# arhix52/Strelka

Hardware: AMD Instinct MI355X
Metric: Mray/s (higher is better)
Workload: dtype f32; 1 GPU; kitchen stand-in (SURVEY 8d C3): 1724134 unique triangles, 2022 instances of 153 meshes, 4 rect + 1 distant light, 60/25/10/5 % diffuse/glossy/metal/glass; resolution=1920x1080, bounces=4, spp=64, tile=32, world_size=1, parallelism=single GPU, rays_per_frame=839862650

## Files before the change

### strelka_amd/csrc/skh_device.h

```cpp
#pragma once
#include <hip/hip_runtime.h>
#include <stdint.h>
#include "skh_libm.h"
#include "skh_lshape.h"

namespace skh
{

struct v3
{
    float x, y, z;
};
struct v4
{
    float x, y, z, w;
};

#define SKH_DI static __device__ __forceinline__

SKH_DI v3 mk3(float x, float y, float z)
{
    v3 r;
    r.x = x;
    r.y = y;
// ... 331 lines not shown
    return norm;
}
SKH_DI void fill_light_data(const Light& l, const v3& hitPoint, LightSample& d)
{
    d.area = calc_light_area(l);
    d.normal = calc_light_normal(l, hitPoint);
    const v3 toLight = d.pointOnLight - hitPoint;
    const float lenToLight = length(toLight);
    d.L = toLight / lenToLight;
    d.distToLight = lenToLight;
}
struct SphQuad
{
    v3 o, x, y, z;
    float z0, z0sq, x0, y0, y0sq, x1, y1, y1sq, b0, b1, b0sq, k, S;
};
SKH_DI SphQuad sph_quad_init(const Light& l, const v3& o)
{
    SphQuad q;
    const v3 ex = mk3(l.points[1]) - mk3(l.points[0]);
    const v3 ey = mk3(l.points[3]) - mk3(l.points[0]);
    const v3 s = mk3(l.points[0]);
    const float exl = length(ex);
    const float eyl = length(ey);
    q.o = o;
    q.x = ex / exl;
    q.y = ey / eyl;
    q.z = cross(q.x, q.y);
    const v3 d = s - o;
    q.z0 = dot(d, q.z);
    if (q.z0 > 0)
    {
        q.z = q.z * -1.0f;
        q.z0 *= -1.0f;
    }
    q.z0sq = q.z0 * q.z0;
    q.x0 = dot(d, q.x);
    q.y0 = dot(d, q.y);
    q.x1 = q.x0 + exl;
    q.y1 = q.y0 + eyl;
    q.y0sq = q.y0 * q.y0;
    q.y1sq = q.y1 * q.y1;
    const v3 v00 = mk3(q.x0, q.y0, q.z0), v01 = mk3(q.x0, q.y1, q.z0), v10 = mk3(q.x1, q.y0, q.z0),
             v11 = mk3(q.x1, q.y1, q.z0);
    const v3 n0 = normalize(cross(v00, v10));
    const v3 n1 = normalize(cross(v10, v11));
    const v3 n2 = normalize(cross(v11, v01));
    const v3 n3 = normalize(cross(v01, v00));
    const float g0 = skm::acosf_(-dot(n0, n1));
    const float g1 = skm::acosf_(-dot(n1, n2));
    const float g2 = skm::acosf_(-dot(n2, n3));
    const float g3 = skm::acosf_(-dot(n3, n0));
    q.b0 = n0.z;
    q.b1 = n2.z;
    q.b0sq = q.b0 * q.b0;
    q.k = 2.0f * SKH_PI - g2 - g3;
    q.S = g0 + g1 - q.k;
    return q;
}
SKH_DI v3 sph_quad_sample(const SphQuad& q, float u, float v)
{
    const float au = u * q.S + q.k;
    const float fu = (skm::cosf_(au) * q.b0 - q.b1) / skm::sinf_(au);
    float cu = 1.0f / sqrtf(fu * fu + q.b0sq) * (fu > 0.0f ? 1.0f : -1.0f);
    cu = clampf(cu, -1.0f, 1.0f);
    float xu = -(cu * q.z0) / sqrtf(1.0f - cu * cu);
    xu = clampf(xu, q.x0, q.x1);
    const float d = sqrtf(xu * xu + q.z0sq);
    const float h0 = q.y0 / sqrtf(d * d + q.y0sq);
    const float h1 = q.y1 / sqrtf(d * d + q.y1sq);
    const float hv = h0 + v * (h1 - h0);
    const float hv2 = hv * hv;
    const float eps = 1e-5f;
    const float yv = (hv < 1.0f - eps) ? (hv * d) / sqrtf(1 - hv2) : q.y1;
    return (q.o + xu * q.x + yv * q.y + q.z0 * q.z);
}
SKH_DI float get_light_pdf(const Light& l, const v3& lightHitPoint, const v3& surfaceHitPoint)
{
    switch (l.type)
    {
    case 0: {
        LightSample d;
        d.pointOnLight = lightHitPoint;
        fill_light_data(l, surfaceHitPoint, d);
        return d.distToLight * d.distToLight / (dot(-d.L, d.normal) * d.area);
    }
    case 2:
        return 1.0f / (4.0f * SKH_PI);
    case 3:
        return 1.0f / (2.0f * SKH_PI * (1.0f - skm::cosf_(l.halfAngle)));
    default:
        break;
    }
    return 0.0f;
}
SKH_DI LightSample sample_rect_light_uniform(const Light& l, float ux, float uy, const v3& hitPoint)
{
    LightSample d;
    const v3 e1 = mk3(l.points[1]) - mk3(l.points[0]);
    const v3 e2 = mk3(l.points[3]) - mk3(l.points[0]);
    d.pointOnLight = mk3(l.points[0]) + e1 * ux + e2 * uy;
    fill_light_data(l, hitPoint, d);
    d.pdf = d.distToLight * d.distToLight / (-dot(d.L, d.normal) * d.area);
    return d;
}
SKH_DI LightSample sample_rect_light(const Light& l, float ux, float uy, const v3& hitPoint)
{
    LightSample d;
    const v3 e1 = mk3(l.points[1]) - mk3(l.points[0]);
    const v3 e2 = mk3(l.points[3]) - mk3(l.points[0]);
    const SphQuad quad = sph_quad_init(l, hitPoint);
    if (quad.S <= 0.0f)
    {
        d.pdf = 0.0f;
        d.pointOnLight = mk3(l.points[0]) + e1 * ux + e2 * uy;
        fill_light_data(l, hitPoint, d);
        return d;
    }
    if (quad.S < 1e-3f)
    {
        d.pointOnLight = mk3(l.points[0]) + e1 * ux + e2 * uy;
        fill_light_data(l, hitPoint, d);
        d.pdf = d.distToLight * d.distToLight / (-dot(d.L, d.normal) * d.area);
        return d;
    }
    d.pointOnLight = sph_quad_sample(quad, ux, uy);
    fill_light_data(l, hitPoint, d);
    d.pdf = 1.0f / quad.S;
    return d;
}
SKH_DI void create_coordinate_system(const v3& N, v3& Nt, v3& Nb)
{
    if (fabsf(N.x) > fabsf(N.y))
    {
        const float invLen = 1.0f / sqrtf(N.x * N.x + N.z * N.z);
        Nt = mk3(-N.z * invLen, 0.0f, N.x * invLen);
    }
    else
    {
        const float invLen = 1.0f / sqrtf(N.y * N.y + N.z * N.z);
        Nt = mk3(0.0f, N.z * invLen, -N.y * invLen);
// ... 543 lines not shown
    EV_ABSORB = 0,
    EV_DIFFUSE = 1,
    EV_GLOSSY = 2,
    EV_SPECULAR = 4,
    EV_REFLECTION = 8,
    EV_TRANSMISSION = 16
};
struct Material
{
    uint32_t type;
    float base_color[3];
    float roughness, metallic, specular, ior;
    uint32_t base_color_texture, normal_texture;
    float reserved[6];
};
struct BsdfSample
{
    v3 k2, bsdf_over_pdf;
    float pdf;
    int event_type;
};
struct BsdfEval
{
    v3 bsdf_diffuse, bsdf_glossy;
    float pdf;
};
SKH_DI v3 cosine_hemisphere(float u1, float u2, float& cosTheta)
{
    const float r = sqrtf(u1);
    const float phi = 2.0f * SKH_PI * u2;
// ... 27 lines not shown
    const v3 T2 = cross(Vh, T1);
    const float r = sqrtf(u1);
    const float phi = 2.0f * SKH_PI * u2;
    const float t1 = r * skm::cosf_(phi);
    float t2 = r * skm::sinf_(phi);
    const float s = 0.5f * (1.0f + Vh.z);
    t2 = (1.0f - s) * sqrtf(fmaxf(0.0f, 1.0f - t1 * t1)) + s * t2;
    const v3 Nh = t1 * T1 + t2 * T2 + sqrtf(fmaxf(0.0f, 1.0f - t1 * t1 - t2 * t2)) * Vh;
    return normalize(mk3(alpha * Nh.x, alpha * Nh.y, fmaxf(0.0f, Nh.z)));
}
struct PbrTerms
{
    v3 diffuse_albedo, f0;
    float alpha, p_spec;
};
SKH_DI PbrTerms pbr_terms(const Material& m)
{
    PbrTerms t;
    const v3 base = mk3(m.base_color[0], m.base_color[1], m.base_color[2]);
    const float metallic = clampf(m.metallic, 0.0f, 1.0f);
    t.diffuse_albedo = base * (1.0f - metallic);
    const float d = 0.08f * m.specular;
    t.f0 = mk3(d) + (base - mk3(d)) * metallic;
    const float r = fmaxf(m.roughness, 0.05f);
    t.alpha = r * r;
    t.p_spec = 0.5f + 0.5f * metallic;
    return t;
}
SKH_DI void pbr_eval_local(const PbrTerms& t, const v3& wo, const v3& wi, v3& fd, v3& fs, float& pdf)
{
    fd = mk3(0.0f);
    fs = mk3(0.0f);
    pdf = 0.0f;
    if (wo.z <= 0.0f || wi.z <= 0.0f)
        return;
    const v3 h = normalize(wo + wi);
    const float oh = fmaxf(dot(wo, h), 0.0f);
    const v3 F = schlick3(t.f0, oh);
    const float D = ggx_D(t.alpha, h.z);
// ... 356 lines not shown
SKH_DI bool hair_frame(const v3& normal, const v3& tangent_u, v3& X, v3& Y, v3& Z)
{
    const float tl = dot(tangent_u, tangent_u);
    if (!(tl > 0.0f))
        return false;
    X = tangent_u * (1.0f / sqrtf(tl));
    const v3 z = normal - X * dot(normal, X);
    const float zl = dot(z, z);
    if (!(zl > 1e-12f))
        return false;
    Z = z * (1.0f / sqrtf(zl));
    Y = cross(Z, X);
    return true;
}

template <bool HAIR>
SKH_DI void bsdf_sample(const Material& m, const v3& stN, const v3& stNg, const v3& stT, const v3& k1, float xi0, float xi1, float xi2,
                        float xi3, bool inside, BsdfSample& out, const HairConst* hc = nullptr )
{
    v3 N = stN, Ng = stNg;
    if (dot(Ng, k1) < 0.0f)
    {
        N = -N;
        Ng = -Ng;
    }
    v3 b1, b2;
    onb_from_z(N, b1, b2);
    const v3 wo = mk3(dot(k1, b1), dot(k1, b2), dot(k1, N));
    out.k2 = mk3(0.0f);
    out.bsdf_over_pdf = mk3(0.0f);
    out.pdf = 0.0f;
    out.event_type = EV_ABSORB;
    const v3 base = mk3(m.base_color[0], m.base_color[1], m.base_color[2]);
    if (m.type == 0)
    {
        float cosT;
        const v3 w = cosine_hemisphere(xi0, xi1, cosT);
        const v3 k2 = normalize(w.x * b1 + w.y * b2 + w.z * N);
        if (cosT <= 0.0f || dot(k2, Ng) <= 0.0f)
            return;
        out.k2 = k2;
        out.pdf = cosT / SKH_PI;
        out.bsdf_over_pdf = base;
        out.event_type = EV_DIFFUSE | EV_REFLECTION;
        return;
    }
    if (HAIR && m.type == 3)
    {
        v3 X, Y, Z;
        if (!hair_frame(stN, stT, X, Y, Z))
            return;
        const HairTerms t = hair_terms(m, *hc);
        const v3 ho = mk3(dot(k1, X), dot(k1, Y), dot(k1, Z));
        float u2 = xi2;
        if (u2 < t.diffuse_w)
        {
            float cosT;
            const v3 w = cosine_hemisphere(xi0, xi1, cosT);
            const v3 k2 = normalize(w.x * b1 + w.y * b2 + w.z * N);
            if (cosT <= 0.0f)
                return;
            const v3 hi = mk3(dot(k2, X), dot(k2, Y), dot(k2, Z));
// ... 50 lines not shown
        if (dot(k2, Ng) <= 0.0f)
            return;
        v3 fd, fs;
        float pdf;
        pbr_eval_local(t, wo, wi, fd, fs, pdf);
        if (!(pdf > 0.0f))
            return;
        out.k2 = k2;
        out.pdf = pdf;
        out.bsdf_over_pdf = (fd + fs) / pdf;
        out.event_type = ev;
        return;
    }
    if (m.type == 2)
    {
        const float n1 = inside ? m.ior : 1.0f;
        const float n2 = inside ? 1.0f : m.ior;
        const float eta = n1 / n2;
        if (m.roughness >= SKH_GLASS_SMOOTH_BELOW)
        {
            if (wo.z <= 0.0f)
                return;
            const float alpha = fmaxf(m.roughness * m.roughness, 1e-4f);
            v3 wi, weight;
            float pdf;
            bool transmitted;
            if (!rough_glass_sample_local(alpha, eta, base, wo, xi0, xi1, xi2, wi, weight, pdf, transmitted))
                return;
            out.k2 = normalize(wi.x * b1 + wi.y * b2 + wi.z * N);
            out.pdf = pdf;
            out.bsdf_over_pdf = weight;
            out.event_type = EV_GLOSSY | (transmitted ? EV_TRANSMISSION : EV_REFLECTION);
            return;
        }
        const float cosi = fminf(fmaxf(wo.z, 0.0f), 1.0f);
        float cost;
        const float F = fresnel_dielectric(cosi, eta, cost);
        if (xi2 < F)
// ... 76 lines not shown
    v3 fh;
    float ph;
    hair_eval_local_g(t, g, ap, apPdf, hi, fh, ph);
    const v3 k2 = normalize(hi.x * X + hi.y * Y + hi.z * Z);
    const float cosN = dot(k2, N);
    const float pd = cosN > 0.0f ? cosN / SKH_PI : 0.0f;
    const float pdf = t.diffuse_w * pd + (1.0f - t.diffuse_w) * ph;
    if (!(pdf > 0.0f) || !(ph > 0.0f))
        return;
    out.k2 = k2;
    out.pdf = pdf;
    out.bsdf_over_pdf = (t.tint * (t.diffuse_w * pd) + fh * (1.0f - t.diffuse_w)) / pdf;
    out.event_type = EV_GLOSSY | EV_REFLECTION;
}

template <bool HAIR>
SKH_DI void bsdf_evaluate(const Material& m, const v3& stN, const v3& stNg, const v3& stT, const v3& k1, const v3& k2, bool inside, BsdfEval& out,
                          const HairConst* hc = nullptr)
{
    v3 N = stN, Ng = stNg;
    if (dot(Ng, k1) < 0.0f)
    {
        N = -N;
        Ng = -Ng;
    }
    out.bsdf_diffuse = mk3(0.0f);
    out.bsdf_glossy = mk3(0.0f);
    out.pdf = 0.0f;
    const v3 base = mk3(m.base_color[0], m.base_color[1], m.base_color[2]);
    if (m.type == 0)
    {
        const float nk2 = dot(N, k2);
        if (nk2 <= 0.0f || dot(Ng, k2) <= 0.0f)
            return;
        out.bsdf_diffuse = base * (nk2 / SKH_PI);
        out.pdf = nk2 / SKH_PI;
        return;
    }
    if (HAIR && m.type == 3)
    {
        v3 X, Y, Z;
        if (!hair_frame(stN, stT, X, Y, Z))
            return;
        const HairTerms t = hair_terms(m, *hc);
        const v3 ho = mk3(dot(k1, X), dot(k1, Y), dot(k1, Z));
        const v3 hi = mk3(dot(k2, X), dot(k2, Y), dot(k2, Z));
        v3 fh;
        float ph;
        hair_eval_local(t, ho, hi, fh, ph);
        const float cosN = dot(k2, N);
        const float pd = cosN > 0.0f ? cosN / SKH_PI : 0.0f;
        out.bsdf_glossy = fh * (1.0f - t.diffuse_w);
        out.bsdf_diffuse = t.tint * (t.diffuse_w * pd);
        out.pdf = t.diffuse_w * pd + (1.0f - t.diffuse_w) * ph;
        return;
    }
    if (m.type == 1)
    {
        v3 b1, b2;
        onb_from_z(N, b1, b2);
        const v3 wo = mk3(dot(k1, b1), dot(k1, b2), dot(k1, N));
        const v3 wi = mk3(dot(k2, b1), dot(k2, b2), dot(k2, N));
        if (dot(Ng, k2) <= 0.0f)
            return;
        const PbrTerms t = pbr_terms(m);
        pbr_eval_local(t, wo, wi, out.bsdf_diffuse, out.bsdf_glossy, out.pdf);
        return;
    }
    if (m.type == 2 && m.roughness >= SKH_GLASS_SMOOTH_BELOW)
    {
        v3 b1, b2;
        onb_from_z(N, b1, b2);
        const v3 wo = mk3(dot(k1, b1), dot(k1, b2), dot(k1, N));
        const v3 wi = mk3(dot(k2, b1), dot(k2, b2), dot(k2, N));
        const float n1 = inside ? m.ior : 1.0f;
        const float n2 = inside ? 1.0f : m.ior;
        rough_glass_eval_local(fmaxf(m.roughness * m.roughness, 1e-4f), n1 / n2, base, wo, wi, out.bsdf_glossy, out.pdf);
    }
}

}
```

### strelka_amd/csrc/skh_kernels.h

```cpp
#pragma once
#include "skh_bvh.h"
#include "skh_env.h"
#include "skh_emit.h"
#include "skh_blend.h"

namespace skh
{

struct DevInstance
{
    float w2o[12];
    int rootRef;
    uint32_t mask;
    uint32_t type;
    uint32_t pad;
};
struct HostInstance
{
    float o2w[12];
    uint32_t type, geom, material, light;
};

#define SKH_WORLD_CURVES 2
#define SKH_SEG_STRIDE 8
// ... 829 lines not shown
#define SKH_SHADE_WAVES(HAIR) ((HAIR) ? 4 : 5)
#endif
enum
{
    SHADE_ANY = 0,
    SHADE_FIRST,
    SHADE_MIDDLE,
    SHADE_LAST
};
#ifndef SKH_SHADE_POSITIONS
#define SKH_SHADE_POSITIONS 1
#endif
#ifndef SKH_SHADE_WAVES_LAST
#define SKH_SHADE_WAVES_LAST(HAIR, EMIT, MTEX, LSHAPE) ((HAIR) || (EMIT) || (MTEX) || (LSHAPE) ? SKH_SHADE_WAVES(HAIR) : 6)
#endif
#define SKH_SHADE_WAVES_AT(HAIR, EMIT, MTEX, LSHAPE, POS) ((POS) == SHADE_LAST ? SKH_SHADE_WAVES_LAST(HAIR, EMIT, MTEX, LSHAPE) : SKH_SHADE_WAVES(HAIR))
#define SKH_SHADE_ATTR(HAIR, EMIT, MTEX, LSHAPE, POS) \
    __attribute__((amdgpu_waves_per_eu(SKH_SHADE_WAVES_AT(HAIR, EMIT, MTEX, LSHAPE, POS), SKH_SHADE_WAVES_AT(HAIR, EMIT, MTEX, LSHAPE, POS))))
#ifndef SKH_SHADE_BLOCK
#define SKH_SHADE_BLOCK 256
#endif
template <bool HAIR, bool ENV, bool EMIT, bool MTEX, int POS>
__global__ void __launch_bounds__(SKH_SHADE_BLOCK) SKH_SHADE_ATTR(HAIR, EMIT, MTEX, false, POS)
    k_shade(DevScene sc, FrameP fp, uint32_t sampleOffset, uint32_t depth , const uint32_t* __restrict__ tileXY, RayQ rq,
            const uint32_t* __restrict__ countPtr, HitQ hq, PathS ps, RayQ nextQ, uint32_t* __restrict__ nextCount, RayQ shadowQ,
            float4* __restrict__ contrib, uint32_t* __restrict__ shadowCount, EnvP env, EmitP emit, MtexP mtex)
{
    constexpr bool LSHAPE = false;
    const LshapeP lsh = { nullptr };
#include "skh_shade_body.inc"
}
// ... 722 lines not shown
```

### strelka_amd/csrc/skh_shade_body.inc

```
    constexpr bool kLast = POS == SHADE_LAST;
    const bool depth0 = POS == SHADE_ANY ? depth == 0u : POS == SHADE_FIRST;
    const bool stateInit = POS == SHADE_MIDDLE ? depth == 0u : depth0;
    const uint32_t numPick = (ENV ? sc.numLights + (env.nee ? 1u : 0u) : sc.numLights) + (EMIT ? (emit.nee ? 1u : 0u) : 0u);
    __shared__ uint32_t s_wave[2 * (SKH_COMPACT_MAX_WAVES + 1)];
    __shared__ uint32_t s_sobol[SKH_SOBOL_LUT_WORDS];
#if SKH_MATERIALS_LDS
    __shared__ float4 s_mat[SKH_MATERIALS_LDS * 4];
#endif
    const uint32_t shard = blockIdx.x & (SKH_SHARDS - 1u), lb = blockIdx.x / SKH_SHARDS;
    const uint32_t n = countPtr[shard * SKH_COUNT_STRIDE];
    if (lb * blockDim.x >= n)
        return;
    const uint32_t il = lb * blockDim.x + threadIdx.x;
    const uint32_t i = shard * rq.region + il;
#ifdef SKH_LANE_PROFILE
    unsigned long long spc[8] = { 0, 0, 0, 0, 0, 0, 0, 0 }, spT = __builtin_readcyclecounter();
#define SKH_SP(k)                                                    \
    {                                                                \
        const unsigned long long t_ = __builtin_readcyclecounter();  \
        spc[k] += t_ - spT;                                          \
        spT = t_;                                                    \
    }
#else
#define SKH_SP(k)
// ... 5 lines not shown
    {
        constexpr int passes = ((SKH_SOBOL_LUT_WORDS / 4) + SKH_SHADE_BLOCK - 1) / SKH_SHADE_BLOCK;
        uint4 lut[passes];
#pragma unroll
        for (int k = 0; k < passes; ++k)
            if ((k + 1) * SKH_SHADE_BLOCK <= SKH_SOBOL_LUT_WORDS / 4 || threadIdx.x + k * SKH_SHADE_BLOCK < SKH_SOBOL_LUT_WORDS / 4)
                lut[k] = reinterpret_cast<const uint4*>(g_sobol_lut)[threadIdx.x + k * SKH_SHADE_BLOCK];
            else
                lut[k] = make_uint4(0u, 0u, 0u, 0u);
#if SKH_MATERIALS_LDS
        float4 mrow = make_float4(0.0f, 0.0f, 0.0f, 0.0f);
        static_assert(SKH_MATERIALS_LDS * 4 <= SKH_SHADE_BLOCK, "one float4 of the material table per thread");
        if (threadIdx.x < SKH_MATERIALS_LDS * 4 && threadIdx.x < sc.numMaterials * 4u)
            mrow = reinterpret_cast<const float4*>(sc.materials)[threadIdx.x];
#endif
#pragma unroll
        for (int k = 0; k < passes; ++k)
            if ((k + 1) * SKH_SHADE_BLOCK <= SKH_SOBOL_LUT_WORDS / 4 || threadIdx.x + k * SKH_SHADE_BLOCK < SKH_SOBOL_LUT_WORDS / 4)
                reinterpret_cast<uint4*>(s_sobol)[threadIdx.x + k * SKH_SHADE_BLOCK] = lut[k];
#if SKH_MATERIALS_LDS
        if (threadIdx.x < SKH_MATERIALS_LDS * 4)
            s_mat[threadIdx.x] = mrow;
#endif
    }
    __syncthreads();
    bool emitNext = false, emitShadow = false;
    v3 nextO = mk3(0.0f), nextD = mk3(0.0f), shO = mk3(0.0f), shD = mk3(0.0f), shC = mk3(0.0f);
    float shTmax = 0.0f;
    if (valid)
    {
        pid = rq.ids()[i];
        rayO = mk3(rq.plane(0)[i], rq.plane(1)[i], rq.plane(2)[i]);
        rayD = mk3(rq.plane(3)[i], rq.plane(4)[i], rq.plane(5)[i]);
        if (hq.primBits != 0u)
        {
            hr0 = *hq.rec16(i);
            const uint32_t w = __float_as_uint(hr0.w);
            hr1.x = __uint_as_float(w == 0xffffffffu ? w : w >> hq.primBits);
            hr1.y = __uint_as_float(w == 0xffffffffu ? w : ((w & ((1u << hq.primBits) - 1u)) | (hq.direct ? SKH_PRIM_DIRECT : 0u)));
        }
        else
            hr0 = hq.rec(i)[0], hr1 = hq.rec(i)[1];
        const float ht = hr0.x, hu = hr0.y, hv = hr0.z;
        const uint32_t hinst = __float_as_uint(hr1.x), hprim = __float_as_uint(hr1.y);
        float* P = ps.base;
        const size_t S = ps.stride;
        v3 throughput = stateInit ? mk3(1.0f) : mk3(P[pid], P[pid + S], P[pid + 2 * S]);
        v3 radiance = mk3(0.0f);
        bool radianceDirty = false;
#define SKH_RADIANCE_LOAD() radiance = mk3(ps.rad()[pid]), radianceDirty = true
        float lastBsdfPdf = stateInit ? 0.0f : P[pid + 6 * S];
        uint32_t flags = stateInit ? 0u : reinterpret_cast<uint32_t*>(P)[pid + 7 * S];
        bool inside = (flags & PF_INSIDE) != 0;
        bool specularBounce = (flags & PF_SPECULAR) != 0;
        uint32_t firstEvent = (flags >> PF_EVENT_SHIFT) & 3u;
        uint32_t px, py;
        const uint32_t sub = pid / fp.numSlots;
        slot_to_pixel(fp, tileXY, pid - sub * fp.numSlots, px, py);
        Sampler smp = init_sampler(px, py, fp.subframeIndex + sampleOffset + sub, fp.sppTotal, 52u);
        smp.depth = POS == SHADE_FIRST ? 0u : depth;
        uint32_t prdDepth = smp.depth;
        v3 origin = rayO, dir = rayD;

        if (hinst == 0xffffffffu)
        {
            if constexpr (ENV)
            {
                const EnvEval ee = env_eval(env, rayD);
                SKH_RADIANCE_LOAD();
                if (depth0 || specularBounce || !env.nee)
                    radiance = radiance + throughput * ee.Le;
                else
                {
                    const float lightPdf = ee.pdf / (float)numPick;
                    const float misWeight = mis_weight_balance(lastBsdfPdf, lightPdf);
                    radiance = radiance + throughput * ee.Le * misWeight;
                }
            }
            else
            {
                const v3 bg = throughput * mk3(0.0f);
                if (!(bg.x == 0.0f && bg.y == 0.0f && bg.z == 0.0f))
                {
                    SKH_RADIANCE_LOAD();
                    radiance = radiance + bg;
                }
            }
            throughput = mk3(0.0f);
            prdDepth = fp.maxDepth;
        }
// ... 6 lines not shown
            float4 tv[3], tx[2];
            const bool txWanted = HAIR || sc.numTextures != 0u;
            tx[0] = tx[1] = make_float4(0.0f, 0.0f, 0.0f, 0.0f);
            {
                const uint32_t recIdx = directTv ? (hprim & ~SKH_PRIM_DIRECT) : 0u;
                const float4* tp = sc.shadeTris + 6 * (size_t)(hq.primBits ? min(recIdx, hq.recClamp) : recIdx);
#pragma unroll
                for (int k = 0; k < 3; ++k)
                    tv[k] = tp[k];
                if (txWanted)
                    tx[0] = tp[3], tx[1] = tp[4];
            }
            asm volatile("" ::"v"(hi.type), "v"(hi.material), "v"(hi.light));
            if (hi.type == 1)
            {
                const uint32_t lidx = hi.light < sc.numLights ? hi.light : 0u;
                const Light& l = sc.lights[lidx];
                const v3 hitPoint = rayO + ht * rayD;
                if constexpr (LSHAPE)
                {
                    const Lshape lse = lshape_fetch(lsh, lidx);
                    const bool sampledDisc = l.type == 1 && (lse.flags & SKH_LSHAPE_SAMPLE_DISC) != 0u;
                    const v3 lightNormal = sampledDisc ? normalize(mk3(l.normal)) : calc_light_normal(l, hitPoint);
                    if (-dot(rayD, lightNormal) > 0.0f)
                    {
                        const v3 Li = mk3(l.color) * lshape_cone(lse, -rayD);
                        SKH_RADIANCE_LOAD();
                        if (depth0 || specularBounce)
                            radiance = radiance + throughput * Li * -dot(rayD, lightNormal);
                        else
                        {
                            const float lightPdf = (sampledDisc ? disc_light_pdf(l, hitPoint, rayO) : get_light_pdf(l, hitPoint, rayO)) / (float)numPick;
                            const float misWeight = mis_weight_balance(lastBsdfPdf, lightPdf);
                            radiance = radiance + throughput * Li * -dot(rayD, lightNormal) * misWeight;
                        }
                    }
                }
                else
                {
                    const v3 lightNormal = calc_light_normal(l, hitPoint);
                    if (-dot(rayD, lightNormal) > 0.0f)
                    {
                        SKH_RADIANCE_LOAD();
                        if (depth0 || specularBounce)
                            radiance = radiance + throughput * mk3(l.color) * -dot(rayD, lightNormal);
                        else
                        {
                            const float lightPdf = get_light_pdf(l, hitPoint, rayO) / (float)numPick;
                            const float misWeight = mis_weight_balance(lastBsdfPdf, lightPdf);
                            radiance = radiance + throughput * mk3(l.color) * -dot(rayD, lightNormal) * misWeight;
                        }
                    }
                }
                throughput = mk3(0.0f);
            }
            else
            {
                const uint32_t mid = hi.material == 0xffffffffu ? 0u : hi.material;
                float4 matLe = make_float4(0.0f, 0.0f, 0.0f, 0.0f);
                if constexpr (EMIT)
                    matLe = emit.Le[mid < emit.numMaterials ? mid : 0u];
                MtexEntry mte;
                if constexpr (MTEX)
                    mte = mtex_entry(mtex, mid < sc.numMaterials ? mid : 0u);
#if SKH_MATERIALS_LDS
                const uint32_t midc = mid < sc.numMaterials ? mid : 0u;
                Material mat;
                if (midc < (uint32_t)SKH_MATERIALS_LDS)
                {
                    const float4 m0 = s_mat[4 * midc], m1 = s_mat[4 * midc + 1], m2 = s_mat[4 * midc + 2], m3 = s_mat[4 * midc + 3];
                    mat.type = __float_as_uint(m0.x), mat.base_color[0] = m0.y, mat.base_color[1] = m0.z, mat.base_color[2] = m0.w;
                    mat.roughness = m1.x, mat.metallic = m1.y, mat.specular = m1.z, mat.ior = m1.w;
                    mat.base_color_texture = __float_as_uint(m2.x), mat.normal_texture = __float_as_uint(m2.y);
                    mat.reserved[0] = m2.z, mat.reserved[1] = m2.w, mat.reserved[2] = m3.x, mat.reserved[3] = m3.y, mat.reserved[4] = m3.z, mat.reserved[5] = m3.w;
                }
                else
                    mat = sc.materials[midc];
#else
                Material mat = sc.materials[mid < sc.numMaterials ? mid : 0u];
#endif
                if (!directTv && hi.type != 2)
                {
                    const float4* tp = sc.shadeTris + 6 * (size_t)(hi.light + hprim);
#pragma unroll
                    for (int k = 0; k < 3; ++k)
                        tv[k] = tp[k];
                    if (txWanted)
                        tx[0] = tp[3], tx[1] = tp[4];
                }
                asm volatile("" ::"v"(mat.type), "v"(tv[0].x), "v"(tv[1].x), "v"(tv[2].x));
                const bool useBase = mat.base_color_texture != 0u && mat.base_color_texture <= sc.numTextures;
                const bool useNormal = mat.normal_texture != 0u && mat.normal_texture <= sc.numTextures;
                bool mtexWanted = false;
                if constexpr (MTEX)
// ... 15 lines not shown
                        matLe.x = Le.x, matLe.y = Le.y, matLe.z = Le.z;
                    }
                    else if (useBase)
                    {
                        const v4 c = tex_lookup_rgba8(sc.texels, sc.texDesc[mat.base_color_texture - 1u], st.u, st.v);
                        mat.base_color[0] = c.x, mat.base_color[1] = c.y, mat.base_color[2] = c.z;
                    }
                    if (useNormal)
                    {
                        const v4 c = tex_lookup_rgba8(sc.texels, sc.texDesc[mat.normal_texture - 1u], st.u, st.v);
                        const v3 ts = mk3(c.x * 2.0f - 1.0f, c.y * 2.0f - 1.0f, c.z * 2.0f - 1.0f);
                        sh.normal = normalize((st.tangent_u * ts.x + st.tangent_v * ts.y) + sh.normal * ts.z);
                    }
                }
                if (fp.debug == 1)
                    radiance = (sh.normal + mk3(1.0f)) * 0.5f, radianceDirty = true;
                else
                {
                    if constexpr (EMIT)
                    {
                        if (hi.type == 0u && matLe.w > 0.0f)
                        {
                            const v3 ne = inside ? -sh.geom_normal : sh.geom_normal;
                            if (-dot(rayD, ne) > 0.0f)
                            {
                                const v3 Le = mk3(matLe.x, matLe.y, matLe.z);
                                SKH_RADIANCE_LOAD();
                                if (depth0 || specularBounce || !emit.nee)
                                    radiance = radiance + throughput * Le;
                                else
                                {
                                    const float lightPdf = emit_pdf(ne, matLe.w * emit.invSumW, sh.position, rayO) / (float)numPick;
                                    const float misWeight = mis_weight_balance(lastBsdfPdf, lightPdf);
                                    radiance = radiance + throughput * Le * misWeight;
                                }
                            }
                        }
                    }
                    const float xi0 = sampler_random_lut(smp, DIM_BSDF0, s_sobol), xi1 = sampler_random_lut(smp, DIM_BSDF1, s_sobol),
                                xi2 = sampler_random_lut(smp, DIM_BSDF2, s_sobol);
                    const float xi3 = HAIR ? sampler_random_lut(smp, DIM_BSDF3, s_sobol) : 0.0f;
                    const v3 k1 = -rayD;
                    BsdfSample bs;
                    SKH_SP(1)
                    v3 toLight = mk3(0.0f);
                    float lightPdf = 0.0f;
                    v3 lrad = mk3(0.0f);
                    bool wantShadow = false;
// ... 31 lines not shown
                                {
                                    const float ux = sampler_random_lut(smp, DIM_LIGHT_X, s_sobol), uy = sampler_random_lut(smp, DIM_LIGHT_Y, s_sobol);
                                    const EnvSample es = env_sample(env, ux, uy);
                                    toLight = es.dir;
                                    if (dot(sh.normal, es.dir) > 0.0f && es.ev.pdf > 0.0f)
                                    {
                                        wantShadow = true;
                                        distToLight = 1e9f;
                                        lightPdf = es.ev.pdf;
                                        lrad = es.ev.Le;
                                    }
                                    lightPdf *= lightSelectionPdf;
                                    return;
                                }
                            }
                            const Light light = sc.lights[lightId];
                            Lshape lse;
                            if constexpr (LSHAPE)
                                lse = lshape_fetch(lsh, lightId);
                            asm volatile("" ::"v"(light.points[0].x), "v"(light.points[1].x), "v"(light.points[2].x), "v"(light.points[3].x),
                                         "v"(light.color.x), "v"(light.normal.x), "v"(light.type));
                            if constexpr (LSHAPE)
                                asm volatile("" ::"v"(lse.flags), "v"(lse.axis.x));
                            const float ux = sampler_random_lut(smp, DIM_LIGHT_X, s_sobol), uy = sampler_random_lut(smp, DIM_LIGHT_Y, s_sobol);
                            LightSample d;
                            d.pointOnLight = mk3(0.0f);
                            d.pdf = 0.0f;
                            d.normal = mk3(0.0f);
                            d.area = 0.0f;
                            d.L = mk3(0.0f);
                            d.distToLight = 0.0f;
                            switch (light.type)
                            {
                            case 0:
                                d = fp.rectMethod == 0 ? sample_rect_light_uniform(light, ux, uy, sh.position) :
                                                         sample_rect_light(light, ux, uy, sh.position);
                                break;
                            case 1:
                                if constexpr (LSHAPE)
                                {
                                    if (lse.flags & SKH_LSHAPE_SAMPLE_DISC)
                                        d = sample_disc_light(light, ux, uy, sh.position);
                                }
                                break;
                            case 2:
                                d = sample_sphere_light(light, ux, uy, sh.position);
                                break;
                            case 3:
                                d = sample_distant_light(light, ux, uy);
                                break;
                            default:
// ... 8 lines not shown
                                wantShadow = true;
                                distToLight = d.distToLight;
                                lightPdf = d.pdf;
                                lrad = 1.0f * Li * saturatef(dot(sh.normal, d.L));
                            }
                            lightPdf *= lightSelectionPdf;
                        }
                    };
                    const bool hairHit = HAIR && mat.type == 3u;
                    BsdfEval evHair;
                    bool evHairDone = false;
                    if (hairHit)
                    {
                        sampleLight();
                        evHairDone = !(isnan3(lrad) || isnan(lightPdf)) && (((dot(toLight, sh.normal) > 0.0f) != inside) && lightPdf != 0.0f);
                        hair_sample_and_evaluate(mat, sh.normal, sh.geom_normal, stT, k1, xi0, xi1, xi2, xi3, sc.hairConst + (mid < sc.numMaterials ? mid : 0u), bs, evHairDone, toLight, evHair);
                    }
                    else
                        bsdf_sample<HAIR>(mat, sh.normal, sh.geom_normal, stT, k1, xi0, xi1, xi2, xi3, inside, bs, HAIR ? sc.hairConst + (mid < sc.numMaterials ? mid : 0u) : nullptr);
                    SKH_SP(2)
                    if (bs.event_type == EV_ABSORB)
                    {
                        if (depth0)
                            firstEvent = 1;
                        throughput = mk3(0.0f);
                    }
                    else
                    {
                        specularBounce = (bs.event_type & EV_SPECULAR) != 0;
                        if (depth0)
                        {
                            if (bs.event_type & EV_DIFFUSE)
                                firstEvent = 2;
                            if (bs.event_type & EV_GLOSSY)
                                firstEvent = 3;
                        }
                        bool errorOut = false;
                        if (bs.event_type & (EV_DIFFUSE | EV_GLOSSY))
                        {
                            if (!hairHit)
                                sampleLight();
                            if (isnan3(lrad) || isnan(lightPdf))
                            {
                                radiance = mk3(10000.0f, 0.0f, 0.0f), radianceDirty = true;
                                throughput = mk3(0.0f);
                                errorOut = true;
                            }
                            else
                            {
                                const bool isNextEventValid = ((dot(toLight, sh.normal) > 0.0f) != inside) && lightPdf != 0.0f;
                                if (isNextEventValid)
                                {
                                    BsdfEval ev;
                                    SKH_SP(3)
                                    if (hairHit)
                                        ev = evHair;
// ... 17 lines not shown
                                        emitShadow = true;
                                    }
                                }
                            }
                        }
                        if (!kLast && !errorOut)
                        {
                            if (bs.event_type & EV_TRANSMISSION)
                            {
                                inside = !inside;
                                origin = offset_ray(sh.position, -sh.geom_normal);
                            }
                            else
                                origin = offset_ray(sh.position, sh.geom_normal);
                            lastBsdfPdf = specularBounce ? 1.0f : bs.pdf;
                            dir = bs.k2;
                            throughput = throughput * bs.bsdf_over_pdf;
                        }
                    }
                }
            }
        }
        SKH_SP(5)
        if constexpr (kLast)
        {
            if (radianceDirty)
                ps.rad()[pid] = make_float4(radiance.x, radiance.y, radiance.z, 0.0f);
        }
        else
        {
// ... 14 lines not shown
                if (fp.debug == 1)
                    alive = false;
            }
            if (alive && prdDepth >= fp.maxDepth)
                alive = false;
            emitNext = alive;
            nextO = origin;
            nextD = dir;
            P[pid] = throughput.x;
            P[pid + S] = throughput.y;
            P[pid + 2 * S] = throughput.z;
            if (radianceDirty)
            {
                ps.rad()[pid] = make_float4(radiance.x, radiance.y, radiance.z, 0.0f);
            }
            P[pid + 6 * S] = lastBsdfPdf;
            reinterpret_cast<uint32_t*>(P)[pid + 7 * S] =
                (inside ? PF_INSIDE : 0u) | (specularBounce ? PF_SPECULAR : 0u) | (firstEvent << PF_EVENT_SHIFT);
        }
#undef SKH_RADIANCE_LOAD
    }
    SKH_SP(6)
    uint32_t ni = 0, si;
    if constexpr (kLast)
        si = block_compact(emitShadow, shadowCount + shard * SKH_COUNT_STRIDE, s_wave, false);
    else
        block_compact2(emitNext, nextCount + shard * SKH_COUNT_STRIDE, emitShadow, shadowCount + shard * SKH_COUNT_STRIDE, s_wave, ni, si);
    ni += shard * nextQ.region;
    si += shard * shadowQ.region;
    if (!kLast && emitNext)
    {
        nextQ.plane(0)[ni] = nextO.x;
        nextQ.plane(1)[ni] = nextO.y;
        nextQ.plane(2)[ni] = nextO.z;
        nextQ.plane(3)[ni] = nextD.x;
// ... 26 lines not shown
```

Before: 6243 Mray/s.

## Stage lights in LDS, defer state loads, reference materials to cut VGPR pressure

Copies up to 16 light records into shared memory per shade block and reads lights by reference instead of copying them into registers. Materials are carried as a pointer with a few cached fields, and the spherical-quad sampler re-derives its frame from the light record instead of keeping it live. In middle-bounce shading, throughput and last BSDF pdf are loaded late, only on the paths that use them, and the pdf is stored only when it was set. The aim is to shorten register live ranges and raise occupancy, at the cost of extra LDS use, a block-wide light preload and repeated loads.

```diff
diff --git a/strelka_amd/csrc/skh_device.h b/strelka_amd/csrc/skh_device.h
--- a/strelka_amd/csrc/skh_device.h
+++ b/strelka_amd/csrc/skh_device.h
@@ -369,6 +369,7 @@
 {
     v3 o, x, y, z;
     float z0, z0sq, x0, y0, y0sq, x1, y1, y1sq, b0, b1, b0sq, k, S;
+    bool flipped;
 };
 SKH_DI SphQuad sph_quad_init(const Light& l, const v3& o)
 {
@@ -384,7 +385,8 @@
     q.z = cross(q.x, q.y);
     const v3 d = s - o;
     q.z0 = dot(d, q.z);
-    if (q.z0 > 0)
+    q.flipped = q.z0 > 0;
+    if (q.flipped)
     {
         q.z = q.z * -1.0f;
         q.z0 *= -1.0f;
@@ -413,13 +415,13 @@
     q.S = g0 + g1 - q.k;
     return q;
 }
-SKH_DI v3 sph_quad_sample(const SphQuad& q, float u, float v)
+SKH_DI void sph_quad_sample_xy(const SphQuad& q, float u, float v, float& xu, float& yv)
 {
     const float au = u * q.S + q.k;
     const float fu = (skm::cosf_(au) * q.b0 - q.b1) / skm::sinf_(au);
     float cu = 1.0f / sqrtf(fu * fu + q.b0sq) * (fu > 0.0f ? 1.0f : -1.0f);
     cu = clampf(cu, -1.0f, 1.0f);
-    float xu = -(cu * q.z0) / sqrtf(1.0f - cu * cu);
+    xu = -(cu * q.z0) / sqrtf(1.0f - cu * cu);
     xu = clampf(xu, q.x0, q.x1);
     const float d = sqrtf(xu * xu + q.z0sq);
     const float h0 = q.y0 / sqrtf(d * d + q.y0sq);
@@ -427,8 +429,29 @@
     const float hv = h0 + v * (h1 - h0);
     const float hv2 = hv * hv;
     const float eps = 1e-5f;
-    const float yv = (hv < 1.0f - eps) ? (hv * d) / sqrtf(1 - hv2) : q.y1;
+    yv = (hv < 1.0f - eps) ? (hv * d) / sqrtf(1 - hv2) : q.y1;
+}
+SKH_DI v3 sph_quad_sample(const SphQuad& q, float u, float v)
+{
+    float xu, yv;
+    sph_quad_sample_xy(q, u, v, xu, yv);
     return (q.o + xu * q.x + yv * q.y + q.z0 * q.z);
+}
+SKH_DI v3 sph_quad_sample_reread(const SphQuad& q, const Light& l0, float u, float v)
+{
+    float xu, yv;
+    sph_quad_sample_xy(q, u, v, xu, yv);
+    const Light* lp = &l0;
+    asm volatile("" : "+v"(lp));
+    const v3 ex = mk3(lp->points[1]) - mk3(lp->points[0]);
+    const v3 ey = mk3(lp->points[3]) - mk3(lp->points[0]);
+    const float exl = length(ex);
+    const float eyl = length(ey);
+    const v3 x = ex / exl, y = ey / eyl;
+    v3 z = cross(x, y);
+    if (q.flipped)
+        z = z * -1.0f;
+    return (q.o + xu * x + yv * y + q.z0 * z);
 }
 SKH_DI float get_light_pdf(const Light& l, const v3& lightHitPoint, const v3& surfaceHitPoint)
 {
@@ -459,6 +482,7 @@
     d.pdf = d.distToLight * d.distToLight / (-dot(d.L, d.normal) * d.area);
     return d;
 }
+template <bool REREAD = false>
 SKH_DI LightSample sample_rect_light(const Light& l, float ux, float uy, const v3& hitPoint)
 {
     LightSample d;
@@ -479,7 +503,7 @@
         d.pdf = d.distToLight * d.distToLight / (-dot(d.L, d.normal) * d.area);
         return d;
     }
-    d.pointOnLight = sph_quad_sample(quad, ux, uy);
+    d.pointOnLight = REREAD ? sph_quad_sample_reread(quad, l, ux, uy) : sph_quad_sample(quad, ux, uy);
     fill_light_data(l, hitPoint, d);
     d.pdf = 1.0f / quad.S;
     return d;
@@ -1053,6 +1077,21 @@
     uint32_t base_color_texture, normal_texture;
     float reserved[6];
 };
+struct MaterialAt
+{
+    uint32_t type;
+    float base_color[3];
+    uint32_t base_color_texture, normal_texture;
+    const Material* at;
+};
+SKH_DI float mat_roughness(const Material& m) { return m.roughness; }
+SKH_DI float mat_metallic(const Material& m) { return m.metallic; }
+SKH_DI float mat_specular(const Material& m) { return m.specular; }
+SKH_DI float mat_ior(const Material& m) { return m.ior; }
+SKH_DI float mat_roughness(const MaterialAt& m) { return m.at->roughness; }
+SKH_DI float mat_metallic(const MaterialAt& m) { return m.at->metallic; }
+SKH_DI float mat_specular(const MaterialAt& m) { return m.at->specular; }
+SKH_DI float mat_ior(const MaterialAt& m) { return m.at->ior; }
 struct BsdfSample
 {
     v3 k2, bsdf_over_pdf;
@@ -1110,15 +1149,16 @@
     v3 diffuse_albedo, f0;
     float alpha, p_spec;
 };
-SKH_DI PbrTerms pbr_terms(const Material& m)
+template <class M>
+SKH_DI PbrTerms pbr_terms(const M& m)
 {
     PbrTerms t;
     const v3 base = mk3(m.base_color[0], m.base_color[1], m.base_color[2]);
-    const float metallic = clampf(m.metallic, 0.0f, 1.0f);
+    const float metallic = clampf(mat_metallic(m), 0.0f, 1.0f);
     t.diffuse_albedo = base * (1.0f - metallic);
-    const float d = 0.08f * m.specular;
+    const float d = 0.08f * mat_specular(m);
     t.f0 = mk3(d) + (base - mk3(d)) * metallic;
-    const float r = fmaxf(m.roughness, 0.05f);
+    const float r = fmaxf(mat_roughness(m), 0.05f);
     t.alpha = r * r;
     t.p_spec = 0.5f + 0.5f * metallic;
     return t;
@@ -1505,8 +1545,8 @@
     return true;
 }
 
-template <bool HAIR>
-SKH_DI void bsdf_sample(const Material& m, const v3& stN, const v3& stNg, const v3& stT, const v3& k1, float xi0, float xi1, float xi2,
+template <bool HAIR, class M>
+SKH_DI void bsdf_sample(const M& m, const v3& stN, const v3& stNg, const v3& stT, const v3& k1, float xi0, float xi1, float xi2,
                         float xi3, bool inside, BsdfSample& out, const HairConst* hc = nullptr )
 {
     v3 N = stN, Ng = stNg;
@@ -1536,7 +1576,8 @@
         out.event_type = EV_DIFFUSE | EV_REFLECTION;
         return;
     }
-    if (HAIR && m.type == 3)
+    if constexpr (HAIR)
+     if (m.type == 3)
     {
         v3 X, Y, Z;
         if (!hair_frame(stN, stT, X, Y, Z))
@@ -1617,14 +1658,14 @@
     }
     if (m.type == 2)
     {
-        const float n1 = inside ? m.ior : 1.0f;
-        const float n2 = inside ? 1.0f : m.ior;
+        const float n1 = inside ? mat_ior(m) : 1.0f;
+        const float n2 = inside ? 1.0f : mat_ior(m);
         const float eta = n1 / n2;
-        if (m.roughness >= SKH_GLASS_SMOOTH_BELOW)
+        if (mat_roughness(m) >= SKH_GLASS_SMOOTH_BELOW)
         {
             if (wo.z <= 0.0f)
                 return;
-            const float alpha = fmaxf(m.roughness * m.roughness, 1e-4f);
+            const float alpha = fmaxf(mat_roughness(m) * mat_roughness(m), 1e-4f);
             v3 wi, weight;
             float pdf;
             bool transmitted;
@@ -1731,8 +1772,8 @@
     out.event_type = EV_GLOSSY | EV_REFLECTION;
 }
 
-template <bool HAIR>
-SKH_DI void bsdf_evaluate(const Material& m, const v3& stN, const v3& stNg, const v3& stT, const v3& k1, const v3& k2, bool inside, BsdfEval& out,
+template <bool HAIR, class M>
+SKH_DI void bsdf_evaluate(const M& m, const v3& stN, const v3& stNg, const v3& stT, const v3& k1, const v3& k2, bool inside, BsdfEval& out,
                           const HairConst* hc = nullptr)
 {
     v3 N = stN, Ng = stNg;
@@ -1754,7 +1795,8 @@
         out.pdf = nk2 / SKH_PI;
         return;
     }
-    if (HAIR && m.type == 3)
+    if constexpr (HAIR)
+     if (m.type == 3)
     {
         v3 X, Y, Z;
         if (!hair_frame(stN, stT, X, Y, Z))
@@ -1784,16 +1826,16 @@
         pbr_eval_local(t, wo, wi, out.bsdf_diffuse, out.bsdf_glossy, out.pdf);
         return;
     }
-    if (m.type == 2 && m.roughness >= SKH_GLASS_SMOOTH_BELOW)
+    if (m.type == 2 && mat_roughness(m) >= SKH_GLASS_SMOOTH_BELOW)
     {
         v3 b1, b2;
         onb_from_z(N, b1, b2);
         const v3 wo = mk3(dot(k1, b1), dot(k1, b2), dot(k1, N));
         const v3 wi = mk3(dot(k2, b1), dot(k2, b2), dot(k2, N));
-        const float n1 = inside ? m.ior : 1.0f;
-        const float n2 = inside ? 1.0f : m.ior;
-        rough_glass_eval_local(fmaxf(m.roughness * m.roughness, 1e-4f), n1 / n2, base, wo, wi, out.bsdf_glossy, out.pdf);
-    }
-}
-
-}
+        const float n1 = inside ? mat_ior(m) : 1.0f;
+        const float n2 = inside ? 1.0f : mat_ior(m);
+        rough_glass_eval_local(fmaxf(mat_roughness(m) * mat_roughness(m), 1e-4f), n1 / n2, base, wo, wi, out.bsdf_glossy, out.pdf);
+    }
+}
+
+}
diff --git a/strelka_amd/csrc/skh_kernels.h b/strelka_amd/csrc/skh_kernels.h
--- a/strelka_amd/csrc/skh_kernels.h
+++ b/strelka_amd/csrc/skh_kernels.h
@@ -867,7 +867,24 @@
 #ifndef SKH_SHADE_WAVES_LAST
 #define SKH_SHADE_WAVES_LAST(HAIR, EMIT, MTEX, LSHAPE) ((HAIR) || (EMIT) || (MTEX) || (LSHAPE) ? SKH_SHADE_WAVES(HAIR) : 6)
 #endif
-#define SKH_SHADE_WAVES_AT(HAIR, EMIT, MTEX, LSHAPE, POS) ((POS) == SHADE_LAST ? SKH_SHADE_WAVES_LAST(HAIR, EMIT, MTEX, LSHAPE) : SKH_SHADE_WAVES(HAIR))
+#ifndef SKH_SHADE_WAVES_FIRST
+#define SKH_SHADE_WAVES_FIRST(HAIR, EMIT, MTEX, LSHAPE) SKH_SHADE_WAVES(HAIR)
+#endif
+#ifndef SKH_SHADE_WAVES_MIDDLE
+#define SKH_SHADE_WAVES_MIDDLE(HAIR, EMIT, MTEX, LSHAPE) SKH_SHADE_WAVES(HAIR)
+#endif
+#define SKH_SHADE_WAVES_AT(HAIR, EMIT, MTEX, LSHAPE, POS)                          \
+    ((POS) == SHADE_LAST   ? SKH_SHADE_WAVES_LAST(HAIR, EMIT, MTEX, LSHAPE) :      \
+     (POS) == SHADE_FIRST  ? SKH_SHADE_WAVES_FIRST(HAIR, EMIT, MTEX, LSHAPE) :     \
+     (POS) == SHADE_MIDDLE ? SKH_SHADE_WAVES_MIDDLE(HAIR, EMIT, MTEX, LSHAPE) :    \
+                             SKH_SHADE_WAVES(HAIR))
+#ifndef SKH_LIGHTS_LDS
+#define SKH_LIGHTS_LDS 16
+#endif
+#ifndef SKH_SHADE_LIGHTS_LDS_AT
+#define SKH_SHADE_LIGHTS_LDS_AT(HAIR, EMIT, MTEX, LSHAPE, POS) ((HAIR) || (EMIT) || (MTEX) || (LSHAPE) ? 0 : SKH_LIGHTS_LDS)
+#endif
+#define SKH_SHADE_LDS_BUDGET (163840 / 6)
 #define SKH_SHADE_ATTR(HAIR, EMIT, MTEX, LSHAPE, POS) \
     __attribute__((amdgpu_waves_per_eu(SKH_SHADE_WAVES_AT(HAIR, EMIT, MTEX, LSHAPE, POS), SKH_SHADE_WAVES_AT(HAIR, EMIT, MTEX, LSHAPE, POS))))
 #ifndef SKH_SHADE_BLOCK
diff --git a/strelka_amd/csrc/skh_shade_body.inc b/strelka_amd/csrc/skh_shade_body.inc
--- a/strelka_amd/csrc/skh_shade_body.inc
+++ b/strelka_amd/csrc/skh_shade_body.inc
@@ -7,6 +7,14 @@
 #if SKH_MATERIALS_LDS
     __shared__ float4 s_mat[SKH_MATERIALS_LDS * 4];
 #endif
+    constexpr int kLightsLds = SKH_SHADE_LIGHTS_LDS_AT(HAIR, EMIT, MTEX, LSHAPE, POS);
+    static_assert(sizeof(Light) == 7 * sizeof(float4), "a light record is seven float4");
+    __shared__ float4 s_light[kLightsLds > 0 ? kLightsLds * 7 : 1];
+    static_assert(kLightsLds == 0 || sizeof(s_wave) + sizeof(s_sobol) + (SKH_MATERIALS_LDS ? SKH_MATERIALS_LDS * 64 : 0) + kLightsLds * sizeof(Light) <= SKH_SHADE_LDS_BUDGET,
+                  "six blocks of k_shade per CU: the Sobol, material and light tables fit a sixth of the LDS");
+    auto lightAt = [&](uint32_t id) -> const Light* {
+        return id < (uint32_t)kLightsLds ? reinterpret_cast<const Light*>(s_light) + id : sc.lights + id;
+    };
     const uint32_t shard = blockIdx.x & (SKH_SHARDS - 1u), lb = blockIdx.x / SKH_SHARDS;
     const uint32_t n = countPtr[shard * SKH_COUNT_STRIDE];
     if (lb * blockDim.x >= n)
@@ -43,6 +51,13 @@
         if (threadIdx.x < SKH_MATERIALS_LDS * 4 && threadIdx.x < sc.numMaterials * 4u)
             mrow = reinterpret_cast<const float4*>(sc.materials)[threadIdx.x];
 #endif
+        float4 lrow = make_float4(0.0f, 0.0f, 0.0f, 0.0f);
+        if constexpr (kLightsLds > 0)
+        {
+            static_assert(kLightsLds * 7 <= SKH_SHADE_BLOCK, "one float4 of the light table per thread");
+            if (threadIdx.x < kLightsLds * 7 && threadIdx.x < sc.numLights * 7u)
+                lrow = reinterpret_cast<const float4*>(sc.lights)[threadIdx.x];
+        }
 #pragma unroll
         for (int k = 0; k < passes; ++k)
             if ((k + 1) * SKH_SHADE_BLOCK <= SKH_SOBOL_LUT_WORDS / 4 || threadIdx.x + k * SKH_SHADE_BLOCK < SKH_SOBOL_LUT_WORDS / 4)
@@ -51,6 +66,9 @@
         if (threadIdx.x < SKH_MATERIALS_LDS * 4)
             s_mat[threadIdx.x] = mrow;
 #endif
+        if constexpr (kLightsLds > 0)
+            if (threadIdx.x < kLightsLds * 7)
+                s_light[threadIdx.x] = lrow;
     }
     __syncthreads();
     bool emitNext = false, emitShadow = false;
@@ -74,11 +92,17 @@
         const uint32_t hinst = __float_as_uint(hr1.x), hprim = __float_as_uint(hr1.y);
         float* P = ps.base;
         const size_t S = ps.stride;
-        v3 throughput = stateInit ? mk3(1.0f) : mk3(P[pid], P[pid + S], P[pid + 2 * S]);
+        constexpr bool kThrLate = POS == SHADE_MIDDLE && kLightsLds > 0;
+#define SKH_THROUGHPUT_LOAD() mk3(P[pid], P[pid + S], P[pid + 2 * S])
+        v3 throughput = kThrLate ? mk3(__builtin_nondeterministic_value(0.0f), __builtin_nondeterministic_value(0.0f), __builtin_nondeterministic_value(0.0f)) :
+                        stateInit ? mk3(1.0f) : SKH_THROUGHPUT_LOAD();
         v3 radiance = mk3(0.0f);
         bool radianceDirty = false;
 #define SKH_RADIANCE_LOAD() radiance = mk3(ps.rad()[pid]), radianceDirty = true
-        float lastBsdfPdf = stateInit ? 0.0f : P[pid + 6 * S];
+        constexpr bool kPdfLate = POS == SHADE_MIDDLE && kLightsLds > 0;
+        float lastBsdfPdf = kPdfLate ? __builtin_nondeterministic_value(0.0f) : stateInit ? 0.0f : P[pid + 6 * S];
+        bool pdfSet = false;
+#define SKH_LAST_PDF() (kPdfLate ? P[pid + 6 * S] : lastBsdfPdf)
         uint32_t flags = stateInit ? 0u : reinterpret_cast<uint32_t*>(P)[pid + 7 * S];
         bool inside = (flags & PF_INSIDE) != 0;
         bool specularBounce = (flags & PF_SPECULAR) != 0;
@@ -93,6 +117,8 @@
 
         if (hinst == 0xffffffffu)
         {
+            if constexpr (kThrLate)
+                throughput = SKH_THROUGHPUT_LOAD();
             if constexpr (ENV)
             {
                 const EnvEval ee = env_eval(env, rayD);
@@ -102,7 +128,7 @@
                 else
                 {
                     const float lightPdf = ee.pdf / (float)numPick;
-                    const float misWeight = mis_weight_balance(lastBsdfPdf, lightPdf);
+                    const float misWeight = mis_weight_balance(SKH_LAST_PDF(), lightPdf);
                     radiance = radiance + throughput * ee.Le * misWeight;
                 }
             }
@@ -139,8 +165,10 @@
             asm volatile("" ::"v"(hi.type), "v"(hi.material), "v"(hi.light));
             if (hi.type == 1)
             {
+                if constexpr (kThrLate)
+                    throughput = SKH_THROUGHPUT_LOAD();
                 const uint32_t lidx = hi.light < sc.numLights ? hi.light : 0u;
-                const Light& l = sc.lights[lidx];
+                const Light& l = kLightsLds > 0 ? *lightAt(lidx) : sc.lights[lidx];
                 const v3 hitPoint = rayO + ht * rayD;
                 if constexpr (LSHAPE)
                 {
@@ -156,7 +184,7 @@
                         else
                         {
                             const float lightPdf = (sampledDisc ? disc_light_pdf(l, hitPoint, rayO) : get_light_pdf(l, hitPoint, rayO)) / (float)numPick;
-                            const float misWeight = mis_weight_balance(lastBsdfPdf, lightPdf);
+                            const float misWeight = mis_weight_balance(SKH_LAST_PDF(), lightPdf);
                             radiance = radiance + throughput * Li * -dot(rayD, lightNormal) * misWeight;
                         }
                     }
@@ -172,7 +200,7 @@
                         else
                         {
                             const float lightPdf = get_light_pdf(l, hitPoint, rayO) / (float)numPick;
-                            const float misWeight = mis_weight_balance(lastBsdfPdf, lightPdf);
+                            const float misWeight = mis_weight_balance(SKH_LAST_PDF(), lightPdf);
                             radiance = radiance + throughput * mk3(l.color) * -dot(rayD, lightNormal) * misWeight;
                         }
                     }
@@ -188,10 +216,18 @@
                 MtexEntry mte;
                 if constexpr (MTEX)
                     mte = mtex_entry(mtex, mid < sc.numMaterials ? mid : 0u);
+                constexpr bool kMatAt = kLightsLds > 0 && SKH_MATERIALS_LDS > 0 && !HAIR && !MTEX;
+                std::conditional_t<kMatAt, MaterialAt, Material> mat;
 #if SKH_MATERIALS_LDS
                 const uint32_t midc = mid < sc.numMaterials ? mid : 0u;
-                Material mat;
-                if (midc < (uint32_t)SKH_MATERIALS_LDS)
+                if constexpr (kMatAt)
+                {
+                    mat.at = midc < (uint32_t)SKH_MATERIALS_LDS ? reinterpret_cast<const Material*>(s_mat) + midc : sc.materials + midc;
+                    mat.type = mat.at->type;
+                    mat.base_color[0] = mat.at->base_color[0], mat.base_color[1] = mat.at->base_color[1], mat.base_color[2] = mat.at->base_color[2];
+                    mat.base_color_texture = mat.at->base_color_texture, mat.normal_texture = mat.at->normal_texture;
+                }
+                else if (midc < (uint32_t)SKH_MATERIALS_LDS)
                 {
                     const float4 m0 = s_mat[4 * midc], m1 = s_mat[4 * midc + 1], m2 = s_mat[4 * midc + 2], m3 = s_mat[4 * midc + 3];
                     mat.type = __float_as_uint(m0.x), mat.base_color[0] = m0.y, mat.base_color[1] = m0.z, mat.base_color[2] = m0.w;
@@ -202,7 +238,7 @@
                 else
                     mat = sc.materials[midc];
 #else
-                Material mat = sc.materials[mid < sc.numMaterials ? mid : 0u];
+                mat = sc.materials[mid < sc.numMaterials ? mid : 0u];
 #endif
                 if (!directTv && hi.type != 2)
                 {
@@ -248,7 +284,11 @@
                     }
                 }
                 if (fp.debug == 1)
+                {
                     radiance = (sh.normal + mk3(1.0f)) * 0.5f, radianceDirty = true;
+                    if constexpr (kThrLate)
+                        throughput = SKH_THROUGHPUT_LOAD();
+                }
                 else
                 {
                     if constexpr (EMIT)
@@ -265,7 +305,7 @@
                                 else
                                 {
                                     const float lightPdf = emit_pdf(ne, matLe.w * emit.invSumW, sh.position, rayO) / (float)numPick;
-                                    const float misWeight = mis_weight_balance(lastBsdfPdf, lightPdf);
+                                    const float misWeight = mis_weight_balance(SKH_LAST_PDF(), lightPdf);
                                     radiance = radiance + throughput * Le * misWeight;
                                 }
                             }
@@ -327,12 +367,16 @@
                                     return;
                                 }
                             }
-                            const Light light = sc.lights[lightId];
+                            Light lightRec;
+                            if constexpr (kLightsLds == 0)
+                                lightRec = sc.lights[lightId];
+                            const Light& light = kLightsLds > 0 ? *lightAt(lightId) : lightRec;
                             Lshape lse;
                             if constexpr (LSHAPE)
                                 lse = lshape_fetch(lsh, lightId);
-                            asm volatile("" ::"v"(light.points[0].x), "v"(light.points[1].x), "v"(light.points[2].x), "v"(light.points[3].x),
-                                         "v"(light.color.x), "v"(light.normal.x), "v"(light.type));
+                            if constexpr (kLightsLds == 0)
+                                asm volatile("" ::"v"(light.points[0].x), "v"(light.points[1].x), "v"(light.points[2].x), "v"(light.points[3].x),
+                                             "v"(light.color.x), "v"(light.normal.x), "v"(light.type));
                             if constexpr (LSHAPE)
                                 asm volatile("" ::"v"(lse.flags), "v"(lse.axis.x));
                             const float ux = sampler_random_lut(smp, DIM_LIGHT_X, s_sobol), uy = sampler_random_lut(smp, DIM_LIGHT_Y, s_sobol);
@@ -347,7 +391,7 @@
                             {
                             case 0:
                                 d = fp.rectMethod == 0 ? sample_rect_light_uniform(light, ux, uy, sh.position) :
-                                                         sample_rect_light(light, ux, uy, sh.position);
+                                                         sample_rect_light<(kLightsLds > 0)>(light, ux, uy, sh.position);
                                 break;
                             case 1:
                                 if constexpr (LSHAPE)
@@ -386,7 +430,8 @@
                     {
                         sampleLight();
                         evHairDone = !(isnan3(lrad) || isnan(lightPdf)) && (((dot(toLight, sh.normal) > 0.0f) != inside) && lightPdf != 0.0f);
-                        hair_sample_and_evaluate(mat, sh.normal, sh.geom_normal, stT, k1, xi0, xi1, xi2, xi3, sc.hairConst + (mid < sc.numMaterials ? mid : 0u), bs, evHairDone, toLight, evHair);
+                        if constexpr (HAIR)
+                            hair_sample_and_evaluate(mat, sh.normal, sh.geom_normal, stT, k1, xi0, xi1, xi2, xi3, sc.hairConst + (mid < sc.numMaterials ? mid : 0u), bs, evHairDone, toLight, evHair);
                     }
                     else
                         bsdf_sample<HAIR>(mat, sh.normal, sh.geom_normal, stT, k1, xi0, xi1, xi2, xi3, inside, bs, HAIR ? sc.hairConst + (mid < sc.numMaterials ? mid : 0u) : nullptr);
@@ -408,10 +453,15 @@
                                 firstEvent = 3;
                         }
                         bool errorOut = false;
+                        if constexpr (kThrLate)
+                            if (!(bs.event_type & (EV_DIFFUSE | EV_GLOSSY)))
+                                throughput = SKH_THROUGHPUT_LOAD();
                         if (bs.event_type & (EV_DIFFUSE | EV_GLOSSY))
                         {
                             if (!hairHit)
                                 sampleLight();
+                            if constexpr (kThrLate)
+                                throughput = SKH_THROUGHPUT_LOAD();
                             if (isnan3(lrad) || isnan(lightPdf))
                             {
                                 radiance = mk3(10000.0f, 0.0f, 0.0f), radianceDirty = true;
@@ -459,6 +509,7 @@
                             else
                                 origin = offset_ray(sh.position, sh.geom_normal);
                             lastBsdfPdf = specularBounce ? 1.0f : bs.pdf;
+                            pdfSet = true;
                             dir = bs.k2;
                             throughput = throughput * bs.bsdf_over_pdf;
                         }
@@ -503,11 +554,14 @@
             {
                 ps.rad()[pid] = make_float4(radiance.x, radiance.y, radiance.z, 0.0f);
             }
-            P[pid + 6 * S] = lastBsdfPdf;
+            if (!kPdfLate || pdfSet)
+                P[pid + 6 * S] = lastBsdfPdf;
             reinterpret_cast<uint32_t*>(P)[pid + 7 * S] =
                 (inside ? PF_INSIDE : 0u) | (specularBounce ? PF_SPECULAR : 0u) | (firstEvent << PF_EVENT_SHIFT);
         }
 #undef SKH_RADIANCE_LOAD
+#undef SKH_LAST_PDF
+#undef SKH_THROUGHPUT_LOAD
     }
     SKH_SP(6)
     uint32_t ni = 0, si;
```

Result: no change. 6236 Mray/s (-0.1%).
